# DHDev0/Stochastic-muzero

Hardware: NVIDIA B200
Metric: mcts_simulations_per_sec (higher is better)
Workload: dtype bf16

## Files before the change

### include/smz.h

```cpp
#ifndef SMZ_H_
#define SMZ_H_

#include <stddef.h>
#include <stdint.h>

#ifdef __cplusplus
extern "C" {
#endif

#define SMZ_ABI_VERSION 2

enum {
  SMZ_OK = 0,
  SMZ_E_INVALID_ARG = -1,
  SMZ_E_CUDA = -2,
  SMZ_E_CAPACITY = -3,
  SMZ_E_STATE = -4
};

enum {
  SMZ_NET_EXTERNAL = 0,
  SMZ_NET_FP32 = 1,
  SMZ_NET_BF16 = 2,
  SMZ_NET_TC32 = 4,
// ... 45 lines not shown
  uint64_t weight_blob_floats;
  uint64_t arena_bytes;
} smz_dims;

typedef struct smz_tree_host {
  int32_t* visit;
  float* value_sum;
  float* reward;
  float* prior;
  int32_t* child_base;
  int32_t* key;
  double* root_prior;
  float minmax[2];
  int32_t n_uniforms;
  int32_t root_to_play;
} smz_tree_host;

int smz_create(const smz_config* cfg, smz_engine** out);
int smz_destroy(smz_engine* e);
int smz_get_dims(const smz_engine* e, smz_dims* out);
const char* smz_last_error(void);

int smz_set_pbc_table(smz_engine* e, const double* table_host, int32_t n_entries);

int smz_set_player_tables(smz_engine* e, const int8_t* sign_host, const int32_t* to_play_host,
                          int32_t n_phases);

int smz_set_weights(smz_engine* e, const float* blob, uint64_t n_floats, int32_t on_device, void* stream);

int smz_set_seed(smz_engine* e, uint64_t seed, uint64_t tree_id_offset, void* stream);
// ... 37 lines not shown
```

### stochastic-muzero_b200/_lib.py

```python
import ctypes as C
import os

_HERE = os.path.dirname(os.path.abspath(__file__))
LIB_PATH = os.path.join(_HERE, "libsmz.so")

SMZ_ABI_VERSION = 2
SMZ_OK, SMZ_E_INVALID_ARG, SMZ_E_CUDA, SMZ_E_CAPACITY, SMZ_E_STATE = 0, -1, -2, -3, -4
NET_EXTERNAL, NET_FP32, NET_BF16, NET_VISION, NET_TC32, NET_F16 = 0, 1, 2, 3, 4, 5
RNG_PHILOX, RNG_TAPE = 0, 1


class smz_config(C.Structure):
    _fields_ = [
        ("abi_version", C.c_int32), ("device", C.c_int32), ("max_trees", C.c_int32),
        ("num_simulations", C.c_int32), ("action_dim", C.c_int32), ("chance_dim", C.c_int32),
        ("max_action_sample", C.c_int32), ("pb_c_base", C.c_int32),
        ("pb_c_init", C.c_double), ("discount", C.c_double), ("root_dirichlet_alpha", C.c_double),
        ("root_exploration_fraction", C.c_double),
        ("obs_dim", C.c_int32), ("state_dim", C.c_int32), ("hidden_dim", C.c_int32),
        ("num_hidden_layers", C.c_int32), ("net_mode", C.c_int32), ("rng_mode", C.c_int32),
        ("lanes_per_tree", C.c_int32), ("record", C.c_int32),
        ("seed", C.c_uint64), ("tree_id_offset", C.c_uint64),
    ]


class smz_dims(C.Structure):
    _fields_ = [
        ("nodes_per_tree", C.c_int32), ("max_children", C.c_int32), ("policy_stride", C.c_int32),
        ("hidden_stride", C.c_int32), ("hidden_slots", C.c_int32), ("path_stride", C.c_int32),
        ("lanes_per_tree", C.c_int32), ("reserved", C.c_int32),
        ("weight_blob_floats", C.c_uint64), ("arena_bytes", C.c_uint64),
    ]


class smz_tree_host(C.Structure):
    _fields_ = [
        ("visit", C.POINTER(C.c_int32)), ("value_sum", C.POINTER(C.c_float)), ("reward", C.POINTER(C.c_float)),
        ("prior", C.POINTER(C.c_float)), ("child_base", C.POINTER(C.c_int32)), ("key", C.POINTER(C.c_int32)),
        ("root_prior", C.POINTER(C.c_double)), ("minmax", C.c_float * 2), ("n_uniforms", C.c_int32),
        ("root_to_play", C.c_int32),
    ]


_P = C.c_void_p
SIGNATURES = {
    "smz_create": (C.c_int, [C.POINTER(smz_config), C.POINTER(_P)]),
    "smz_destroy": (C.c_int, [_P]),
    "smz_get_dims": (C.c_int, [_P, C.POINTER(smz_dims)]),
    "smz_last_error": (C.c_char_p, []),
    "smz_set_pbc_table": (C.c_int, [_P, C.POINTER(C.c_double), C.c_int32]),
    "smz_set_player_tables": (C.c_int, [_P, C.POINTER(C.c_int8), C.POINTER(C.c_int32), C.c_int32]),
    "smz_set_weights": (C.c_int, [_P, _P, C.c_uint64, C.c_int32, _P]),
    "smz_set_seed": (C.c_int, [_P, C.c_uint64, C.c_uint64, _P]),
    "smz_set_uniform_tape": (C.c_int, [_P, _P, C.c_int32]),
    "smz_root": (C.c_int, [_P, C.c_int32, _P, _P, _P, C.c_int32, _P, _P]),
# ... 32 lines not shown
```

### stochastic-muzero_b200/csrc/smz_api.cu

```cuda
#include <cuda_runtime.h>
#include <math.h>
#include <stdarg.h>
#include <stdio.h>
#include <stdlib.h>
#include <string.h>

#include <vector>

#include "../../include/smz.h"
#include "smz_kernels.h"
#include "smz_net_bf16.h"
#include "smz_net_tc32.h"
#include "smz_net_vision.h"

static thread_local char g_err[512] = "";

static int fail(int code, const char* fmt, ...) {
  va_list ap;
  va_start(ap, fmt);
  vsnprintf(g_err, sizeof(g_err), fmt, ap);
  va_end(ap);
  return code;
}

// ... 138 lines not shown
  a.one_minus_frac_f32 = (float)(1.0 - c.root_exploration_fraction);
  a.frac = c.root_exploration_fraction;
  a.alpha = c.root_dirichlet_alpha;

  e->dims.nodes_per_tree = a.M; e->dims.max_children = a.Kmax; e->dims.policy_stride = a.W;
  e->dims.hidden_stride = a.Sp; e->dims.hidden_slots = a.N + 1; e->dims.path_stride = a.path_stride;
  e->dims.lanes_per_tree = lanes;
  e->cfg.lanes_per_tree = lanes;

  const size_t B = a.B, M = a.M;
  a.row_cap = (a.B + 511) / 512 * 512 + 512;
  a.row_top = a.row_cap;
  const size_t RC = a.row_cap;
  cudaError_t r = cudaSuccess;
#define ALLOC(ptr, n) if (r == cudaSuccess) r = dev_alloc(e, &(ptr), (n))
  ALLOC(a.stat, B * M); ALLOC(a.link, B * M); ALLOC(a.root_prior, B * a.A); ALLOC(a.minmax, B);
  ALLOC(a.ucursor, B); ALLOC(a.root_to_play, B); ALLOC(a.path, B * a.path_stride); ALLOC(a.path_len, B);
  ALLOC(a.leaf_node, B); ALLOC(a.leaf_slot, B); ALLOC(a.leaf_action, B); ALLOC(a.leaf_branch, B);
  ALLOC(a.branch_count, (size_t)(a.N + 1) * 2); ALLOC(a.rows, 2 * RC); ALLOC(a.rows4, 2 * RC); ALLOC(a.error_flag, 1);
  ALLOC(a.depth_sum, 1);
  a.xin_q = c.net_mode == SMZ_NET_TC32 ? 16 : 8;
  if (c.net_mode == SMZ_NET_BF16 || c.net_mode == SMZ_NET_TC32 || c.net_mode == SMZ_NET_F16) { ALLOC(a.xin, 2 * RC * a.xin_q); }
  if (getenv("SMZ_TREE_TIMELINE")) { ALLOC(a.dbg, 8 + 4 * ((size_t)a.N + 2)); }
  ALLOC(a.out_policy, B * a.W); ALLOC(a.out_value, B); ALLOC(a.out_reward, B); ALLOC(a.dirichlet, B * a.A);
  if (c.record) {
    ALLOC(a.rec_policy, B * a.N * a.W); ALLOC(a.rec_value, B * a.N); ALLOC(a.rec_reward, B * a.N);
    ALLOC(a.rec_branch, B * a.N); ALLOC(a.rec_root_policy, B * a.W);
  }
  ALLOC(e->pbc_dev, (size_t)a.N + 2);
  ALLOC(e->rcp64_dev, (size_t)rcp_entries(a.N));
  ALLOC(e->rcp32_dev, (size_t)rcp_entries(a.N));
  ALLOC(e->seed_dev, 2);
  ALLOC(e->sign_dev, (size_t)a.N + 2);
  if (c.net_mode == SMZ_NET_VISION) {
    ALLOC(a.hidden, (size_t)(a.N + 1) * B * a.Sp);
    e->dims.weight_blob_floats = smz_vision_blob_floats(a.A, c.state_dim, c.hidden_dim, c.num_hidden_layers);
    ALLOC(e->blob_buf, e->dims.weight_blob_floats);
  } else if (c.net_mode != SMZ_NET_EXTERNAL) {
// ... 50 lines not shown
      double tree = 0, net = 0, g1 = 0, g2 = 0;
      int n = 0;
      for (int s = e->a.N - 11; s <= e->a.N - 2; ++s, ++n) {
        const unsigned long long *c = &w[4 * s], *nx = &w[4 * (s + 1)];
        net += (double)(c[3] - c[2]);
        g1 += (double)((long long)c[0] - (long long)c[3]);
        tree += (double)(c[1] - c[0]);
        g2 += (double)((long long)nx[2] - (long long)c[1]);
      }
      fprintf(stderr, "smz step timeline (%%globaltimer, mean of %d simulations): network step %.2f us | -> tree step %.2f us | tree step %.2f us | -> network step %.2f us\n",
              n, net / n / 1e3, g1 / n / 1e3, tree / n / 1e3, g2 / n / 1e3);
    }
    if (cudaMemcpy(t, e->a.dbg, sizeof(t), cudaMemcpyDeviceToHost) == cudaSuccess)
      fprintf(stderr, "smz tree timeline (block 0, last fused launch): expand+backup %lld cycles | descent %lld cycles = %lld levels walked by warp 0 in %lld + leaf record / row reservation %lld (path length of tree 0: %lld)\n",
              t[1] - t[0], t[2] - t[1], t[5], t[4] - t[1], t[2] - t[4], t[3]);
  }
  if (e->graph_exec) cudaGraphExecDestroy(e->graph_exec);
  if (e->capture_stream) cudaStreamDestroy(e->capture_stream);
  if (e->bf16) smz_bf16_destroy(e->bf16);
  if (e->tc32) smz_tc32_destroy(e->tc32);
  if (e->vision) smz_vision_destroy(e->vision);
  for (void* p : e->allocs) cudaFree(p);
  delete e;
  return SMZ_OK;
}

int smz_get_dims(const smz_engine* e, smz_dims* out) {
  if (!e || !out) return fail(SMZ_E_INVALID_ARG, "smz_get_dims: null argument");
  *out = e->dims;
  return SMZ_OK;
// ... 78 lines not shown

int smz_root(smz_engine* e, int32_t n_trees, const float* obs, const float* root_policy, const int32_t* root_to_play,
             int32_t train, const double* dirichlet, void* stream) {
  if (!e) return fail(SMZ_E_INVALID_ARG, "smz_root: null engine");
  if (n_trees < 1 || n_trees > e->a.B) return fail(SMZ_E_CAPACITY, "smz_root: n_trees %d not in [1, %d]", n_trees, e->a.B);
  if ((obs == nullptr) == (root_policy == nullptr))
    return fail(SMZ_E_INVALID_ARG, "smz_root: give exactly one of obs_dev / root_policy_dev");
  if (obs && e->cfg.net_mode == SMZ_NET_EXTERNAL) return fail(SMZ_E_STATE, "smz_root: obs given but engine has no network");
  if (obs && !e->have_weights) return fail(SMZ_E_STATE, "smz_root: smz_set_weights has not been called");
  if (e->cfg.rng_mode == SMZ_RNG_TAPE && !e->a.tape_u) return fail(SMZ_E_STATE, "smz_root: no uniform tape set");
  cudaStream_t s = (cudaStream_t)stream;
  ON_DEVICE(e);
  SmzArena& a = e->a;
  smz_launch_begin_search(a, s);
  if (a.dbg) {
    std::vector<unsigned long long> init(4 * ((size_t)a.N + 2));
    for (size_t i = 0; i < init.size(); ++i) init[i] = (i & 1) ? 0ull : ~0ull;
    CU(cudaMemcpyAsync(a.dbg + 8, init.data(), init.size() * sizeof(init[0]), cudaMemcpyHostToDevice, s));
    CU(cudaStreamSynchronize(s));
  }
  e->launches = 0;
  if (e->cfg.num_simulations == 0) train = 0;
  const float* policy = root_policy;
  if (obs) {
    if (e->vision) { smz_vision_root(e->vision, a, n_trees, obs, s); count_launches(e, 1); }
    else if (e->bf16) smz_bf16_root(e->bf16, a, e->shape, n_trees, obs, s);
    else if (e->tc32) smz_tc32_root(e->tc32, a, e->shape, n_trees, obs, s);
    else smz_net_f32_root(a, e->shape, e->img32, n_trees, obs, s);
    count_launches(e, 1);
    policy = a.out_policy;
  }
  if (train) {
// ... 187 lines not shown
  CU(cudaGetLastError());
  return SMZ_OK;
}

int smz_export_tree(smz_engine* e, int32_t tree, smz_tree_host* out, void* stream) {
  if (!e || !out) return fail(SMZ_E_INVALID_ARG, "smz_export_tree: null argument");
  if (tree < 0 || tree >= e->n_trees) return fail(SMZ_E_INVALID_ARG, "smz_export_tree: tree %d not in [0, %d)", tree, e->n_trees);
  ON_DEVICE(e);
  CU(cudaStreamSynchronize((cudaStream_t)stream));
  const SmzArena& a = e->a;
  const size_t M = a.M;
  std::vector<int4> stat(M);
  std::vector<int2> link(M);
  CU(cudaMemcpy(stat.data(), a.stat + (size_t)tree * M, M * sizeof(int4), cudaMemcpyDeviceToHost));
  CU(cudaMemcpy(link.data(), a.link + (size_t)tree * M, M * sizeof(int2), cudaMemcpyDeviceToHost));
  for (size_t n = 0; n < M; ++n) {
    if (out->visit) out->visit[n] = stat[n].x;
    if (out->value_sum) memcpy(&out->value_sum[n], &stat[n].y, 4);
    if (out->reward) memcpy(&out->reward[n], &stat[n].z, 4);
    if (out->prior) memcpy(&out->prior[n], &stat[n].w, 4);
    if (out->child_base) out->child_base[n] = link[n].x;
    if (out->key) out->key[n] = link[n].y;
  }
  if (out->root_prior)
    CU(cudaMemcpy(out->root_prior, a.root_prior + (size_t)tree * a.A, a.A * sizeof(double), cudaMemcpyDeviceToHost));
  float2 mm;
  CU(cudaMemcpy(&mm, a.minmax + tree, sizeof(mm), cudaMemcpyDeviceToHost));
  out->minmax[0] = mm.x; out->minmax[1] = mm.y;
  CU(cudaMemcpy(&out->n_uniforms, a.ucursor + tree, sizeof(int), cudaMemcpyDeviceToHost));
  CU(cudaMemcpy(&out->root_to_play, a.root_to_play + tree, sizeof(int), cudaMemcpyDeviceToHost));
// ... 56 lines not shown
```

### stochastic-muzero_b200/csrc/smz_common.cuh

```cuda
#pragma once
#include <cuda_runtime.h>
#include <stdint.h>

#define SMZ_BRANCH_AFTERSTATE 0
#define SMZ_BRANCH_DYNAMICS 1
#define SMZ_MAX_POLICY 32
#define SMZ_HP 128
#define SMZ_SP 64
#define SMZ_VISION_SP 160

struct SmzArena {
  int B, N, A, C, K, Kd, Kc, Kmax, M, W, Sp, path_stride, n_phases;
  int row_cap, row_top;
  int4* stat;
  int2* link;
  double* root_prior;
  float2* minmax;
  int* ucursor;
  int* root_to_play;
  int4* path;
  int* path_len;
  int* leaf_node;
  int* leaf_slot;
  int* leaf_action;
  int* leaf_branch;
  int* branch_count;
  int* rows;
  int4* rows4;
  uint4* xin;
  int xin_q;
// ... 18 lines not shown
  const double* rcp64;
  const float* rcp32;
  const signed char* sign;
  float discount;
  float one_minus_frac_f32;
  double frac;
  double alpha;
};

#ifdef __CUDACC__
__device__ __forceinline__ unsigned long long smz_globaltimer() {
  unsigned long long t;
  asm volatile("mov.u64 %0, %%globaltimer;" : "=l"(t));
  return t;
}
__device__ __forceinline__ void smz_stamp_min(long long* dbg, int sim, int k) {
  if (dbg && threadIdx.x == 0) atomicMin(reinterpret_cast<unsigned long long*>(dbg) + 8 + 4 * sim + k, smz_globaltimer());
}
__device__ __forceinline__ void smz_stamp_max(long long* dbg, int sim, int k) {
  if (dbg && threadIdx.x == 0) atomicMax(reinterpret_cast<unsigned long long*>(dbg) + 8 + 4 * sim + k, smz_globaltimer());
}
__device__ __forceinline__ size_t smz_row_index(const SmzArena& a, int sim, int branch, int row) {
  return (size_t)(sim & 1) * a.row_cap + (branch ? a.row_top - 1 - row : row);
}
__device__ __forceinline__ void smz_pdl_wait() { asm volatile("griddepcontrol.wait;" ::: "memory"); }
__device__ __forceinline__ void smz_pdl_launch_dependents() { asm volatile("griddepcontrol.launch_dependents;" ::: "memory"); }

template <typename... KArgs, typename... Args>
inline cudaError_t smz_launch(void (*kernel)(KArgs...), dim3 grid, dim3 block, size_t smem, cudaStream_t s, bool pdl,
                              Args... args) {
// ... 63 lines not shown
```

### stochastic-muzero_b200/csrc/smz_tree.cu

```cuda
#include <stdlib.h>

#include "smz_common.cuh"
#include "smz_kernels.h"
#include "smz_tree_dev.cuh"

namespace {

using namespace smz_tree_dev;

template <int G>
__global__ void k_root_expand(SmzArena a, int n_trees, const float* __restrict__ policy, int pstride,
                              const int* __restrict__ root_to_play, int train,
                              const double* __restrict__ dirichlet) {
  Group<G> g;
  int tree = (blockIdx.x * blockDim.x + threadIdx.x) / G;
  const bool alive = tree < n_trees;
  if (!alive) tree = n_trees - 1;
  const size_t tb = (size_t)tree * a.M;
  const int n = a.A;
  int cursor = 0;
  const float pol = (g.gl < n) ? policy[(size_t)tree * pstride + g.gl] : 0.f;
  const float p = normalise_policy(g, pol, n);
  const SmzRng rng = smz_make_rng(a);
  choice_without_replacement(g, a, rng, alive, tree, p, n, n, cursor);
  if (!alive) return;
  if (g.gl < n) {
    double prior = (double)p;
    if (train) {
      const double nz = dirichlet[(size_t)tree * a.A + g.gl];
      prior = __dadd_rn((double)__fmul_rn(p, a.one_minus_frac_f32), __dmul_rn(nz, a.frac));
    }
    a.root_prior[(size_t)tree * a.A + g.gl] = prior;
    a.stat[tb + 1 + g.gl] = make_int4(0, 0, 0, __float_as_int(p));
    a.link[tb + 1 + g.gl] = make_int2(0, g.gl);
  }
  if (g.gl == 0) {
    a.stat[tb] = make_int4(0, 0, 0, 0);
    a.link[tb] = make_int2(1, -1);
    a.minmax[tree] = make_float2(__int_as_float(0x7f800000), __int_as_float(0xff800000));
    a.ucursor[tree] = cursor;
    const int rtp = root_to_play ? root_to_play[tree] % a.n_phases : 0;
    a.root_to_play[tree] = rtp < 0 ? rtp + a.n_phases : rtp;
    a.path_len[tree] = 0;
    if (a.rec_root_policy)
      for (int i = 0; i < a.W; ++i) a.rec_root_policy[(size_t)tree * a.W + i] = i < n ? policy[(size_t)tree * pstride + i] : 0.f;
  }
}

template <int G>
__global__ void k_select(SmzArena a, int n_trees, int sim, int* __restrict__ o_slot, int* __restrict__ o_action,
                         int* __restrict__ o_branch) {
  Group<G> g;
// ... 8 lines not shown
  ts.root = make_int2(rs.x, rs.y);
  select_phase<G, true, false, true>(g, a, rng, tree, alive, sim, ts, o_slot, o_action, o_branch);
}

template <int G>
__global__ void k_expand_backup(SmzArena a, int n_trees, int sim, const float* __restrict__ policy, int pstride,
                                const float* __restrict__ value, const float* __restrict__ reward) {
  Group<G> g;
  int tree = (blockIdx.x * blockDim.x + threadIdx.x) / G;
  const bool alive = tree < n_trees;
  if (!alive) tree = n_trees - 1;
  const SmzRng rng = smz_make_rng(a);
  expand_backup_phase(g, a, rng, tree, alive, sim, policy, pstride, value, reward);
}

template <int G>
__global__ void k_backup_select(SmzArena a, int n_trees, int sim) {
  smz_pdl_wait();
  smz_pdl_launch_dependents();
  Group<G> g;
  int tree = (blockIdx.x * blockDim.x + threadIdx.x) / G;
  const bool alive = tree < n_trees;
  if (!alive) tree = n_trees - 1;
  const bool stamp = a.dbg && blockIdx.x == 0 && threadIdx.x == 0;
  if (stamp) a.dbg[0] = clock64();
  const SmzRng rng = smz_make_rng(a);
  const TreeState ts = expand_backup_phase(g, a, rng, tree, alive, sim, a.out_policy, a.W, a.out_value, a.out_reward);
  __syncwarp();
  if (stamp) a.dbg[1] = clock64();
  select_phase<G, true, false, true>(g, a, rng, tree, alive, sim + 1, ts, nullptr, nullptr, nullptr);
  if (stamp) { a.dbg[2] = clock64(); a.dbg[3] = a.path_len[tree]; }
}

constexpr int SMZ_UWIN = 32;

__host__ __device__ inline size_t smz_mirror_bytes(int tpb, int M, int A, int n_tab, int n_pbc) {
  size_t b = (size_t)tpb * M * (sizeof(int4) + sizeof(int2));
  b += (size_t)tpb * (A + SMZ_UWIN) * sizeof(double);
  b += (size_t)(n_pbc + n_tab) * sizeof(double) + (size_t)n_tab * sizeof(float);
  return b + 16;
}

template <int G>
__global__ void k_backup_select_sm(SmzArena a, int n_trees, int sim, int n_tab) {
  extern __shared__ int4 smz_sm_nodes[];
  Group<G> g;
  int tree = (blockIdx.x * blockDim.x + threadIdx.x) / G;
  const bool alive = tree < n_trees;
  if (!alive) tree = n_trees - 1;
  const int tpb = blockDim.x / G, lt = threadIdx.x / G;
  int4* sst = smz_sm_nodes + (size_t)lt * a.M;
  int2* slk_all = reinterpret_cast<int2*>(smz_sm_nodes + (size_t)tpb * a.M);
  int2* slk = slk_all + (size_t)lt * a.M;
  double* dbl = reinterpret_cast<double*>(slk_all + (size_t)tpb * a.M + ((size_t)tpb * a.M & 1));
  double* srp = dbl + (size_t)lt * a.A;
  double* swin = dbl + (size_t)tpb * a.A + (size_t)lt * SMZ_UWIN;
  double* spbc = dbl + (size_t)tpb * (a.A + SMZ_UWIN);
  double* sr64 = spbc + (a.N + 2);
  float* sr32 = reinterpret_cast<float*>(sr64 + n_tab);

  SmzRng rng = smz_make_rng(a);
  const int cursor0 = a.ucursor[tree];
  {
    const size_t tb = (size_t)tree * a.M;
    const int used = 1 + a.A + sim * a.Kmax;
    for (int i = g.gl; i < used; i += G) {
      sst[i] = a.stat[tb + i];
      slk[i] = a.link[tb + i];
    }
    for (int i = g.gl; i < a.A; i += G) srp[i] = a.root_prior[(size_t)tree * a.A + i];
    for (int i = threadIdx.x; i < a.N + 2; i += blockDim.x) spbc[i] = a.pbc[i];
    for (int i = threadIdx.x; i < n_tab; i += blockDim.x) { sr64[i] = a.rcp64[i]; sr32[i] = a.rcp32[i]; }
    if (rng.mode == 0)
      for (int i = g.gl; i < SMZ_UWIN; i += G) swin[i] = smz_rng_uniform(rng, tree, cursor0 + i);
  }
  SmzArena al = a;
  al.pbc = spbc; al.rcp64 = sr64; al.rcp32 = sr32;
  if (rng.mode == 0) { rng.win = swin; rng.win_base = cursor0; rng.win_len = SMZ_UWIN; }
  smz_pdl_wait();
  smz_pdl_launch_dependents();
  smz_stamp_min(a.dbg, sim, 0);
  __syncthreads();
  const bool stamp = a.dbg && blockIdx.x == 0 && threadIdx.x == 0;
  if (stamp) a.dbg[0] = clock64();
  const TreeState ts = expand_backup_phase<G, true>(g, al, rng, tree, alive, sim, a.out_policy, a.W, a.out_value, a.out_reward,
                                                    sst, slk);
  __syncwarp();
  if (stamp) a.dbg[1] = clock64();
  select_phase<G, true, true, true>(g, al, rng, tree, alive, sim + 1, ts, nullptr, nullptr, nullptr, sst, slk, srp);
  if (stamp) { a.dbg[2] = clock64(); a.dbg[3] = a.path_len[tree]; }
  if (a.dbg) {
    __syncthreads();
    smz_stamp_max(a.dbg, sim, 1);
  }
}

__global__ void k_read_roots(SmzArena a, int n_trees, int* __restrict__ visits, float* __restrict__ values,
                             double* __restrict__ priors, float* __restrict__ rewards, int* __restrict__ error_out) {
  const int i = blockIdx.x * blockDim.x + threadIdx.x;
  if (i == 0 && error_out) *error_out = *a.error_flag;
  if (i >= n_trees * a.A) return;
  const int tree = i / a.A, c = i % a.A;
  const size_t tb = (size_t)tree * a.M;
  const int4 st = a.stat[tb + 1 + c];
// ... 124 lines not shown
                              const float* value, const float* reward, cudaStream_t s) {
  SMZ_DISPATCH_G(lanes, (k_expand_backup<G><<<grid_for<G>(n_trees, kThreads), kThreads, 0, s>>>(
                            a, n_trees, sim, policy, pstride, value, reward)));
}

static int rcp_entries(const SmzArena& a) { return a.N + 3 > SMZ_MAX_POLICY + 1 ? a.N + 3 : SMZ_MAX_POLICY + 1; }
static size_t mirror_bytes(const SmzArena& a, int lanes) {
  return smz_mirror_bytes(kThreads / lanes, a.M, a.A, rcp_entries(a), a.N + 2);
}

bool smz_tree_mirror_fits(const SmzArena& a, int lanes) {
  const bool off = getenv("SMZ_NO_TREE_SMEM") != nullptr;
  return !off && mirror_bytes(a, lanes) <= 96 * 1024;
}

static bool mirror_pays(int blocks) {
  static int sms_of[64] = {0};
  int dev = 0;
  cudaGetDevice(&dev);
  int& sms = sms_of[dev & 63];
  if (!sms && (cudaDeviceGetAttribute(&sms, cudaDevAttrMultiProcessorCount, dev) != cudaSuccess || sms <= 0)) sms = 148;
  static const int per_sm = getenv("SMZ_MIRROR_BLOCKS_PER_SM") ? atoi(getenv("SMZ_MIRROR_BLOCKS_PER_SM")) : 2;
  return blocks <= per_sm * sms;
}

void smz_launch_backup_select(const SmzArena& a, int lanes, int n_trees, int sim, bool pdl, cudaStream_t s) {
  if (smz_tree_mirror_fits(a, lanes) && mirror_pays((n_trees * lanes + kThreads - 1) / kThreads)) {
    const size_t smem = mirror_bytes(a, lanes);
    SMZ_DISPATCH_G(lanes, (cudaFuncSetAttribute((const void*)k_backup_select_sm<G>, cudaFuncAttributeMaxDynamicSharedMemorySize,
                                                (int)smem),
                           getenv("SMZ_NO_CARVEOUT") ? cudaSuccess :
                           cudaFuncSetAttribute((const void*)k_backup_select_sm<G>, cudaFuncAttributePreferredSharedMemoryCarveout,
                                                cudaSharedmemCarveoutMaxShared),
                           smz_launch(k_backup_select_sm<G>, dim3(grid_for<G>(n_trees, kThreads)), dim3(kThreads), smem, s, pdl,
                                      a, n_trees, sim, rcp_entries(a))));
    return;
  }
  SMZ_DISPATCH_G(lanes, (smz_launch(k_backup_select<G>, dim3(grid_for<G>(n_trees, kThreads)), dim3(kThreads), 0, s, pdl,
                                    a, n_trees, sim)));
}

void smz_launch_read_roots(const SmzArena& a, int n_trees, int* visits, float* values, double* priors, float* rewards,
                           int* error_out, cudaStream_t s) {
  const int n = n_trees * a.A;
  k_read_roots<<<(n + 255) / 256, 256, 0, s>>>(a, n_trees, visits, values, priors, rewards, error_out);
}

void smz_launch_select_actions(const SmzArena& a, int n_trees, double temperature, const double* u, int* actions,
                               double* policy, double* stored, cudaStream_t s) {
  k_select_actions<<<(n_trees + 127) / 128, 128, 0, s>>>(a, n_trees, temperature, u, actions, policy, stored);
}

__global__ void k_begin_search(SmzArena a) {
  for (int i = threadIdx.x; i < (a.N + 1) * 2; i += blockDim.x) a.branch_count[i] = 0;
// ... 16 lines not shown
```

### stochastic-muzero_b200/csrc/smz_tree_dev.cuh

```cuda
#pragma once
#include "smz_common.cuh"

namespace smz_tree_dev {

#define FULL 0xffffffffu

template <int G>
struct Group {
  int lane, gl, gbase;
  __device__ Group() {
    lane = threadIdx.x & 31;
    gl = lane & (G - 1);
    gbase = lane & ~(G - 1);
  }
  template <typename T>
  __device__ T bcast(T v, int src) const { return __shfl_sync(FULL, v, src, G); }
  __device__ unsigned ballot(bool p) const {
    unsigned b = __ballot_sync(FULL, p);
    return (G == 32) ? b : ((b >> gbase) & ((1u << G) - 1u));
  }
};

template <int G>
__device__ float np_sum_f32(const Group<G>& g, float a, int n) {
// ... 97 lines not shown
#pragma unroll
      for (int i = 0; i < G; ++i) cnt += g.bcast(c, i) <= u;
    }
  }
  return cnt;
}

template <int G>
__device__ float normalise_policy(const Group<G>& g, float pol, int n) {
  const float p = (g.gl < n) ? __fadd_rn(pol, 1e-12f) : 0.f;
  const float s = np_sum_f32(g, p, n);
  return (g.gl < n) ? __fdiv_rn(p, s) : 0.f;
}

template <int G>
__device__ unsigned choice_without_replacement(const Group<G>& g, const SmzArena& a, const SmzRng& rng, bool alive, int tree,
                                               float p32, int n, int bound, int& cursor) {
  unsigned found = 0;
  int nf = alive ? 0 : bound;
  if (g.ballot(alive && g.gl < n && !(p32 >= 0.f))) {
    if (alive) *a.error_flag = 2;
    found = bound >= 32 ? 0xffffffffu : ((1u << bound) - 1u);
    nf = bound;
  }
  const double pd = (g.gl < n) ? (double)p32 : 0.0;
  for (int round = 0; __any_sync(FULL, nf < bound); ++round) {
    if (round > 2 * SMZ_MAX_POLICY) {
      if (nf < bound) {
        *a.error_flag = 2;
        for (int i = 0; i < n && nf < bound; ++i)
// ... 16 lines not shown
    for (int off = G / 2; off > 0; off >>= 1) bits |= __shfl_xor_sync(FULL, bits, off, G);
    found |= bits;
    nf = alive ? __popc(found) : bound;
    cursor += m;
  }
  return found;
}


struct TreeState {
  int cursor;
  float2 mm;
  int2 root;
};

template <int G, bool COMPACT = true, bool MIRROR = false, bool BLOCKAGG = false>
__device__ __forceinline__ void select_phase(const Group<G>& g, const SmzArena& a, const SmzRng& rng, int tree, bool alive,
                                             int sim, TreeState ts, int* __restrict__ o_slot, int* __restrict__ o_action,
                                             int* __restrict__ o_branch, const int4* __restrict__ sst = nullptr,
                                             const int2* __restrict__ slk = nullptr, const double* __restrict__ srp = nullptr) {
  const size_t tb = (size_t)tree * a.M;
  int cursor = ts.cursor;
  const float vmin = ts.mm.x, vmax = ts.mm.y;
  int4* path = a.path + (size_t)tree * a.path_stride;

  int depth = 0, cbase = 1, nch = a.A;
  int parent_visit = ts.root.x;
  const float range = __fsub_rn(vmax, vmin);
  const float rrange = vmax > vmin ? __frcp_rn(range) : 0.f;
  const bool range_plain = (__float_as_int(range) & 0x7FFFFF) == 0x7FFFFF || range < 1e-30f;
  if (alive && g.gl == 0) path[0] = make_int4(0, ts.root.x, ts.root.y, 0);
  int L = 1, child = 0, child_key = 0;
  bool going = alive;
  const double prior0 = (alive && g.gl < a.A) ? (srp ? srp[g.gl] : a.root_prior[(size_t)tree * a.A + g.gl]) : 0.0;
  int level = 0;
  while (__any_sync(FULL, going)) {
    const bool act = going && g.gl < nch;
    const bool chance = (level >> 1) & 1;
    const int ci = act ? cbase + g.gl : 0;
    int4 st;
    int2 lk;
    if constexpr (MIRROR) {
      st = sst[ci];
      lk = slk[ci];
    } else {
      st = a.stat[tb + ci];
      lk = a.link[tb + ci];
    }
    if (!act) { st = make_int4(0, 0, 0, 0); lk = make_int2(0, 0); }
    const double pbc = chance ? 0.0 : a.pbc[going ? parent_visit : 0];
    const int uidx = chance ? cursor : cursor + g.gl;
    const bool want = going && (chance || act);
    const unsigned wofs = (unsigned)(uidx - rng.win_base);
    const bool hit = rng.win != nullptr && wofs < (unsigned)rng.win_len;
    double u = hit ? rng.win[wofs] : 0.0;
    if (__any_sync(FULL, want && !hit)) {
      if (want && !hit) u = smz_rng_uniform(rng, tree, uidx);
    }
    int pick = 0;
    if (chance) {
      const float p = __int_as_float(st.w);
      const float om = act ? __fadd_rn(__fsub_rn(1.f, p), 1e-12f) : 0.f;
      const float rem = fabsf(smz_div_r32(np_sum_f32(g, om, nch), (float)nch, a.rcp32[nch]));
      const float sh = act ? __fadd_rn(p, rem) : 0.f;
      const float tot = np_sum_f32(g, sh, nch);
      const float q = act ? __fdiv_rn(sh, tot) : 0.f;
      double total;
      const double num = choice_cdf_raw(g, (double)q, nch, total);
      const float cf = cdf_f32(num, total, act), uf = (float)u;
      bool le = cf < uf;
      const bool close = act && fabsf(cf - uf) <= SMZ_CDF_MARGIN;
      if (__any_sync(FULL, close)) {
        if (close) le = __ddiv_rn(num, total) <= u;
      }
      int pk = __popc(g.ballot(act && le));
      pk = pk < nch ? pk : nch - 1;
      if (chance) { pick = pk; cursor += going ? 1 : 0; }
    }
    if (!chance) {
      double score = -__longlong_as_double(0x7ff0000000000000LL);
      int best = -1;
      if (act && !chance) {
        const double prior = (level == 0) ? prior0 : (double)__int_as_float(st.w);
        const double ps = smz_div_r64(__dmul_rn(pbc, prior), (double)(st.x + 1), a.rcp64[st.x + 1]);
        double vs = 0.0;
        if (st.x > 0) {
          const float val = smz_div_r32(__int_as_float(st.y), (float)st.x, a.rcp32[st.x]);
// ... 18 lines not shown
    const int key = g.bcast(lk.y, pick);
    if (going) {
      child = cbase + pick;
      child_key = key;
      if (g.gl == 0) path[L] = make_int4(child, cst.x, cst.y, cst.z);
      ++L;
      if (child_cb == 0 || L >= a.path_stride) {
        going = false;
      } else {
        nch = chance ? a.Kd : a.Kc;
        parent_visit = cst.x;
        cbase = child_cb;
        ++depth;
      }
    }
    ++level;
  }
  if (a.dbg && blockIdx.x == 0 && threadIdx.x == 0) { a.dbg[4] = clock64(); a.dbg[5] = level; }
  const bool lead = alive && g.gl == 0;
  const int branch = ((depth >> 1) & 1) ? SMZ_BRANCH_DYNAMICS : SMZ_BRANCH_AFTERSTATE;
  const int slot = (cbase == 1) ? 0 : (cbase - 1 - a.A) / a.Kmax + 1;
  uint4 hcopy[(G < 8) ? 8 / G : 1], hcopy2[(G < 8) ? 8 / G : 1];
  const bool copy_row = COMPACT && a.xin != nullptr && alive;
  const bool wide_row = a.xin_q > 8;
  if (copy_row) {
    const uint4* src = reinterpret_cast<const uint4*>(a.hidden) + ((size_t)slot * a.B + tree) * a.xin_q;
#pragma unroll
    for (int j = 0; j < ((G < 8) ? 8 / G : 1); ++j) {
      const int idx = g.gl + j * G;
      hcopy[j] = idx < 8 ? src[idx] : make_uint4(0, 0, 0, 0);
      if (wide_row) hcopy2[j] = idx < 8 ? src[8 + idx] : make_uint4(0, 0, 0, 0);
// ... 87 lines not shown
  float2 mm = a.minmax[tree];
  float v = value[tree];
  const float rew_in = reward[tree];
  const signed char* sign = a.sign + (size_t)a.root_to_play[tree] * (a.N + 2);

  const int n = branch ? a.A : a.C;
  const int bound = min(a.K, n);
  const float pol = (g.gl < n) ? policy[(size_t)tree * pstride + g.gl] : 0.f;
  const float p = normalise_policy(g, pol, n);
  const unsigned found = choice_without_replacement(g, a, rng, alive, tree, p, n, bound, cursor);
  const int cb = 1 + a.A + sim * a.Kmax;
  if (alive && g.gl < n && ((found >> g.gl) & 1u)) {
    const int r = __popc(found & ((1u << g.gl) - 1u));
    a.stat[tb + cb + r] = make_int4(0, 0, 0, __float_as_int(p));
    a.link[tb + cb + r] = make_int2(0, g.gl);
    if constexpr (MIRROR) {
      sst[cb + r] = make_int4(0, 0, 0, __float_as_int(p));
      slk[cb + r] = make_int2(0, g.gl);
    }
  }
  const float rew = branch ? rew_in : 0.f;
  if (alive && g.gl == 0) {
    a.link[tb + leaf].x = cb;
    a.ucursor[tree] = cursor;
    if (branch) reinterpret_cast<int*>(a.stat + tb + leaf)[2] = __float_as_int(rew);
    if constexpr (MIRROR) {
      slk[leaf].x = cb;
      if (branch) sst[leaf].z = __float_as_int(rew);
    }
    if (a.rec_policy) {
// ... 67 lines not shown
```

### stochastic-muzero_b200/engine.py

```python
from __future__ import annotations

import ctypes as C
from typing import Dict, Optional

import numpy as np
import torch

from . import _lib
from .weights import VISION_FLAT, ModelShape, VisionShape

SEARCH_KEYS = ("pb_c_base", "pb_c_init", "discount", "root_dirichlet_alpha", "root_exploration_fraction",
               "num_simulations", "maxium_action_sample", "number_of_player", "custom_loop")
_NET = {"external": _lib.NET_EXTERNAL, "fp32": _lib.NET_FP32, "bf16": _lib.NET_BF16, "vision": _lib.NET_VISION,
        "tc32": _lib.NET_TC32, "f16": _lib.NET_F16}
_RNG = {"philox": _lib.RNG_PHILOX, "tape": _lib.RNG_TAPE}


class SmzError(RuntimeError):
    pass


def _is_chance(depth: int) -> bool:
    return bool((depth >> 1) & 1)

# ... 273 lines not shown
               "dirichlet": self._new(n, A, dtype=torch.float64), "root_policy": self._new(n, W, dtype=torch.float32)}
        self._check(self.lib.smz_read_record(self._h, self._ptr(rec["sim_policy"]), self._ptr(rec["sim_value"]),
                                             self._ptr(rec["sim_reward"]), self._ptr(rec["sim_branch"]),
                                             self._ptr(rec["dirichlet"]), self._ptr(rec["root_policy"]), self._stream))
        return rec

    def stats(self):
        depth, launches, total = C.c_double(), C.c_int64(), C.c_int64()
        self._check(self.lib.smz_stats(self._h, C.byref(depth), C.byref(launches), C.byref(total), self._stream))
        return {"mean_leaf_depth": depth.value, "launches": launches.value, "launches_total": total.value}

    def export_arena(self, tree: int) -> Dict[str, np.ndarray]:
        M, A = self.dims.nodes_per_tree, self.A
        cols = {"visit": np.zeros(M, np.int32), "value_sum": np.zeros(M, np.float32), "reward": np.zeros(M, np.float32),
                "prior": np.zeros(M, np.float32), "child_base": np.zeros(M, np.int32), "key": np.zeros(M, np.int32),
                "root_prior": np.zeros(A, np.float64)}
        th = _lib.smz_tree_host()
        th.visit = cols["visit"].ctypes.data_as(C.POINTER(C.c_int32))
        th.value_sum = cols["value_sum"].ctypes.data_as(C.POINTER(C.c_float))
        th.reward = cols["reward"].ctypes.data_as(C.POINTER(C.c_float))
        th.prior = cols["prior"].ctypes.data_as(C.POINTER(C.c_float))
        th.child_base = cols["child_base"].ctypes.data_as(C.POINTER(C.c_int32))
        th.key = cols["key"].ctypes.data_as(C.POINTER(C.c_int32))
        th.root_prior = cols["root_prior"].ctypes.data_as(C.POINTER(C.c_double))
        self._check(self.lib.smz_export_tree(self._h, int(tree), C.byref(th), self._stream))
        cols["minmax"] = np.array([th.minmax[0], th.minmax[1]], np.float32)
        cols["n_uniforms"] = int(th.n_uniforms)
        cols["root_to_play"] = int(th.root_to_play)
        return cols

    def n_children(self, depth: int) -> int:
        if depth == 0:
            return self.A
        return min(self.K, self.A) if _is_chance(depth - 1) else min(self.K, self.Cdim)

    def export_tree(self, tree: int) -> Dict[str, np.ndarray]:
        ar = self.export_arena(tree)
        phase = ar["root_to_play"] % self.n_phases
        rows = []
# ... 17 lines not shown
```

Baseline: 187.3 million.

## Precompute and store chance-node CDFs instead of recomputing per descent

Adds a per-node cdf array. On expansion each chance child set gets a marker, and a fill pass at the start of backup_select computes the normalized chance CDF once. Later descents read the stored value instead of redoing two group reductions and a scan at every chance level. Values close to the margin are still recomputed exactly, and a heuristic picks the stored path only when the lane count or block count suggests it pays. The change also adds per-level timeline instrumentation behind the debug flag, plus extra memory and writes for the cdf array.

Result: faster. 190.3 million (median of 6 runs) (+1.6%).

```diff
diff --git a/include/smz.h b/include/smz.h
--- a/include/smz.h
+++ b/include/smz.h
@@ -83,6 +83,7 @@
   float minmax[2];
   int32_t n_uniforms;
   int32_t root_to_play;
+  float* cdf;
 } smz_tree_host;
 
 int smz_create(const smz_config* cfg, smz_engine** out);
diff --git a/stochastic-muzero_b200/_lib.py b/stochastic-muzero_b200/_lib.py
--- a/stochastic-muzero_b200/_lib.py
+++ b/stochastic-muzero_b200/_lib.py
@@ -38,7 +38,7 @@
         ("visit", C.POINTER(C.c_int32)), ("value_sum", C.POINTER(C.c_float)), ("reward", C.POINTER(C.c_float)),
         ("prior", C.POINTER(C.c_float)), ("child_base", C.POINTER(C.c_int32)), ("key", C.POINTER(C.c_int32)),
         ("root_prior", C.POINTER(C.c_double)), ("minmax", C.c_float * 2), ("n_uniforms", C.c_int32),
-        ("root_to_play", C.c_int32),
+        ("root_to_play", C.c_int32), ("cdf", C.POINTER(C.c_float)),
     ]
 
 
diff --git a/stochastic-muzero_b200/csrc/smz_api.cu b/stochastic-muzero_b200/csrc/smz_api.cu
--- a/stochastic-muzero_b200/csrc/smz_api.cu
+++ b/stochastic-muzero_b200/csrc/smz_api.cu
@@ -176,14 +176,14 @@
   const size_t RC = a.row_cap;
   cudaError_t r = cudaSuccess;
 #define ALLOC(ptr, n) if (r == cudaSuccess) r = dev_alloc(e, &(ptr), (n))
-  ALLOC(a.stat, B * M); ALLOC(a.link, B * M); ALLOC(a.root_prior, B * a.A); ALLOC(a.minmax, B);
+  ALLOC(a.stat, B * M); ALLOC(a.link, B * M); ALLOC(a.cdf, B * M); ALLOC(a.root_prior, B * a.A); ALLOC(a.minmax, B);
   ALLOC(a.ucursor, B); ALLOC(a.root_to_play, B); ALLOC(a.path, B * a.path_stride); ALLOC(a.path_len, B);
   ALLOC(a.leaf_node, B); ALLOC(a.leaf_slot, B); ALLOC(a.leaf_action, B); ALLOC(a.leaf_branch, B);
   ALLOC(a.branch_count, (size_t)(a.N + 1) * 2); ALLOC(a.rows, 2 * RC); ALLOC(a.rows4, 2 * RC); ALLOC(a.error_flag, 1);
   ALLOC(a.depth_sum, 1);
   a.xin_q = c.net_mode == SMZ_NET_TC32 ? 16 : 8;
   if (c.net_mode == SMZ_NET_BF16 || c.net_mode == SMZ_NET_TC32 || c.net_mode == SMZ_NET_F16) { ALLOC(a.xin, 2 * RC * a.xin_q); }
-  if (getenv("SMZ_TREE_TIMELINE")) { ALLOC(a.dbg, 8 + 4 * ((size_t)a.N + 2)); }
+  if (getenv("SMZ_TREE_TIMELINE")) { ALLOC(a.dbg, smz_tl_levels_base(a) + 8 * ((size_t)a.N + 2)); }
   ALLOC(a.out_policy, B * a.W); ALLOC(a.out_value, B); ALLOC(a.out_reward, B); ALLOC(a.dirichlet, B * a.A);
   if (c.record) {
     ALLOC(a.rec_policy, B * a.N * a.W); ALLOC(a.rec_value, B * a.N); ALLOC(a.rec_reward, B * a.N);
@@ -264,6 +264,12 @@
     if (cudaMemcpy(t, e->a.dbg, sizeof(t), cudaMemcpyDeviceToHost) == cudaSuccess)
       fprintf(stderr, "smz tree timeline (block 0, last fused launch): expand+backup %lld cycles | descent %lld cycles = %lld levels walked by warp 0 in %lld + leaf record / row reservation %lld (path length of tree 0: %lld)\n",
               t[1] - t[0], t[2] - t[1], t[5], t[4] - t[1], t[2] - t[4], t[3]);
+    unsigned long long q[8];
+    if (e->a.N >= 2 && cudaMemcpy(q, e->a.dbg + smz_tl_levels_base(e->a) + 8 * (e->a.N - 1), sizeof(q), cudaMemcpyDeviceToHost) == cudaSuccess &&
+        q[4] > 0)
+      fprintf(stderr, "smz tree levels (descent of simulation %d, all %llu warps): decision %.0f cycles/level over %llu levels | chance %.0f cycles/level over %llu levels | mean %.2f levels per warp | deepest warp %llu levels | slowest warp descent %llu cycles\n",
+              e->a.N - 1, q[4], q[1] ? (double)q[0] / q[1] : 0.0, q[1], q[3] ? (double)q[2] / q[3] : 0.0, q[3],
+              (double)(q[1] + q[3]) / q[4], q[5], q[6]);
   }
   if (e->graph_exec) cudaGraphExecDestroy(e->graph_exec);
   if (e->capture_stream) cudaStreamDestroy(e->capture_stream);
@@ -372,8 +378,8 @@
   SmzArena& a = e->a;
   smz_launch_begin_search(a, s);
   if (a.dbg) {
-    std::vector<unsigned long long> init(4 * ((size_t)a.N + 2));
-    for (size_t i = 0; i < init.size(); ++i) init[i] = (i & 1) ? 0ull : ~0ull;
+    std::vector<unsigned long long> init(12 * ((size_t)a.N + 2), 0ull);
+    for (size_t i = 0; i < 4 * ((size_t)a.N + 2); ++i) init[i] = (i & 1) ? 0ull : ~0ull;
     CU(cudaMemcpyAsync(a.dbg + 8, init.data(), init.size() * sizeof(init[0]), cudaMemcpyHostToDevice, s));
     CU(cudaStreamSynchronize(s));
   }
@@ -591,6 +597,7 @@
   std::vector<int2> link(M);
   CU(cudaMemcpy(stat.data(), a.stat + (size_t)tree * M, M * sizeof(int4), cudaMemcpyDeviceToHost));
   CU(cudaMemcpy(link.data(), a.link + (size_t)tree * M, M * sizeof(int2), cudaMemcpyDeviceToHost));
+  if (out->cdf) CU(cudaMemcpy(out->cdf, a.cdf + (size_t)tree * M, M * sizeof(float), cudaMemcpyDeviceToHost));
   for (size_t n = 0; n < M; ++n) {
     if (out->visit) out->visit[n] = stat[n].x;
     if (out->value_sum) memcpy(&out->value_sum[n], &stat[n].y, 4);
diff --git a/stochastic-muzero_b200/csrc/smz_common.cuh b/stochastic-muzero_b200/csrc/smz_common.cuh
--- a/stochastic-muzero_b200/csrc/smz_common.cuh
+++ b/stochastic-muzero_b200/csrc/smz_common.cuh
@@ -14,6 +14,7 @@
   int row_cap, row_top;
   int4* stat;
   int2* link;
+  float* cdf;
   double* root_prior;
   float2* minmax;
   int* ucursor;
@@ -62,6 +63,7 @@
   asm volatile("mov.u64 %0, %%globaltimer;" : "=l"(t));
   return t;
 }
+__host__ __device__ __forceinline__ size_t smz_tl_levels_base(const SmzArena& a) { return 8 + 4 * ((size_t)a.N + 2); }
 __device__ __forceinline__ void smz_stamp_min(long long* dbg, int sim, int k) {
   if (dbg && threadIdx.x == 0) atomicMin(reinterpret_cast<unsigned long long*>(dbg) + 8 + 4 * sim + k, smz_globaltimer());
 }
diff --git a/stochastic-muzero_b200/csrc/smz_tree.cu b/stochastic-muzero_b200/csrc/smz_tree.cu
--- a/stochastic-muzero_b200/csrc/smz_tree.cu
+++ b/stochastic-muzero_b200/csrc/smz_tree.cu
@@ -33,9 +33,11 @@
     a.root_prior[(size_t)tree * a.A + g.gl] = prior;
     a.stat[tb + 1 + g.gl] = make_int4(0, 0, 0, __float_as_int(p));
     a.link[tb + 1 + g.gl] = make_int2(0, g.gl);
+    a.cdf[tb + 1 + g.gl] = p;
   }
   if (g.gl == 0) {
     a.stat[tb] = make_int4(0, 0, 0, 0);
+    a.cdf[tb] = 0.f;
     a.link[tb] = make_int2(1, -1);
     a.minmax[tree] = make_float2(__int_as_float(0x7f800000), __int_as_float(0xff800000));
     a.ucursor[tree] = cursor;
@@ -74,21 +76,22 @@
   expand_backup_phase(g, a, rng, tree, alive, sim, policy, pstride, value, reward);
 }
 
-template <int G>
+template <int G, bool STORED>
 __global__ void k_backup_select(SmzArena a, int n_trees, int sim) {
+  Group<G> g;
+  int tree = (blockIdx.x * blockDim.x + threadIdx.x) / G;
+  const bool alive = tree < n_trees;
+  if (!alive) tree = n_trees - 1;
+  if (STORED) fill_chance_cdf(g, a, tree, alive, sim);
   smz_pdl_wait();
   smz_pdl_launch_dependents();
-  Group<G> g;
-  int tree = (blockIdx.x * blockDim.x + threadIdx.x) / G;
-  const bool alive = tree < n_trees;
-  if (!alive) tree = n_trees - 1;
   const bool stamp = a.dbg && blockIdx.x == 0 && threadIdx.x == 0;
   if (stamp) a.dbg[0] = clock64();
   const SmzRng rng = smz_make_rng(a);
   const TreeState ts = expand_backup_phase(g, a, rng, tree, alive, sim, a.out_policy, a.W, a.out_value, a.out_reward);
   __syncwarp();
   if (stamp) a.dbg[1] = clock64();
-  select_phase<G, true, false, true>(g, a, rng, tree, alive, sim + 1, ts, nullptr, nullptr, nullptr);
+  select_phase<G, true, false, true, STORED>(g, a, rng, tree, alive, sim + 1, ts, nullptr, nullptr, nullptr);
   if (stamp) { a.dbg[2] = clock64(); a.dbg[3] = a.path_len[tree]; }
 }
 
@@ -101,7 +104,7 @@
   return b + 16;
 }
 
-template <int G>
+template <int G, bool STORED>
 __global__ void k_backup_select_sm(SmzArena a, int n_trees, int sim, int n_tab) {
   extern __shared__ int4 smz_sm_nodes[];
   Group<G> g;
@@ -124,8 +127,12 @@
   {
     const size_t tb = (size_t)tree * a.M;
     const int used = 1 + a.A + sim * a.Kmax;
+    if (STORED) fill_chance_cdf(g, a, tree, alive, sim);
+    __syncwarp();
     for (int i = g.gl; i < used; i += G) {
-      sst[i] = a.stat[tb + i];
+      int4 st = a.stat[tb + i];
+      if (STORED) st.w = __float_as_int(a.cdf[tb + i]);
+      sst[i] = st;
       slk[i] = a.link[tb + i];
     }
     for (int i = g.gl; i < a.A; i += G) srp[i] = a.root_prior[(size_t)tree * a.A + i];
@@ -147,7 +154,7 @@
                                                     sst, slk);
   __syncwarp();
   if (stamp) a.dbg[1] = clock64();
-  select_phase<G, true, true, true>(g, al, rng, tree, alive, sim + 1, ts, nullptr, nullptr, nullptr, sst, slk, srp);
+  select_phase<G, true, true, true, STORED>(g, al, rng, tree, alive, sim + 1, ts, nullptr, nullptr, nullptr, sst, slk, srp);
   if (stamp) { a.dbg[2] = clock64(); a.dbg[3] = a.path_len[tree]; }
   if (a.dbg) {
     __syncthreads();
@@ -302,30 +309,41 @@
   return !off && mirror_bytes(a, lanes) <= 96 * 1024;
 }
 
-static bool mirror_pays(int blocks) {
+static int device_sms() {
   static int sms_of[64] = {0};
   int dev = 0;
   cudaGetDevice(&dev);
   int& sms = sms_of[dev & 63];
   if (!sms && (cudaDeviceGetAttribute(&sms, cudaDevAttrMultiProcessorCount, dev) != cudaSuccess || sms <= 0)) sms = 148;
+  return sms;
+}
+static bool mirror_pays(int blocks) {
   static const int per_sm = getenv("SMZ_MIRROR_BLOCKS_PER_SM") ? atoi(getenv("SMZ_MIRROR_BLOCKS_PER_SM")) : 2;
-  return blocks <= per_sm * sms;
-}
-
-void smz_launch_backup_select(const SmzArena& a, int lanes, int n_trees, int sim, bool pdl, cudaStream_t s) {
-  if (smz_tree_mirror_fits(a, lanes) && mirror_pays((n_trees * lanes + kThreads - 1) / kThreads)) {
+  return blocks <= per_sm * device_sms();
+}
+static bool stored_cdf_pays(int lanes, int blocks) { return lanes >= 16 || 2 * blocks <= 3 * device_sms(); }
+
+template <bool STORED>
+static void launch_backup_select(const SmzArena& a, int lanes, int n_trees, int sim, bool pdl, int blocks, cudaStream_t s) {
+  if (smz_tree_mirror_fits(a, lanes) && mirror_pays(blocks)) {
     const size_t smem = mirror_bytes(a, lanes);
-    SMZ_DISPATCH_G(lanes, (cudaFuncSetAttribute((const void*)k_backup_select_sm<G>, cudaFuncAttributeMaxDynamicSharedMemorySize,
+    SMZ_DISPATCH_G(lanes, (cudaFuncSetAttribute((const void*)k_backup_select_sm<G, STORED>, cudaFuncAttributeMaxDynamicSharedMemorySize,
                                                 (int)smem),
                            getenv("SMZ_NO_CARVEOUT") ? cudaSuccess :
-                           cudaFuncSetAttribute((const void*)k_backup_select_sm<G>, cudaFuncAttributePreferredSharedMemoryCarveout,
+                           cudaFuncSetAttribute((const void*)k_backup_select_sm<G, STORED>, cudaFuncAttributePreferredSharedMemoryCarveout,
                                                 cudaSharedmemCarveoutMaxShared),
-                           smz_launch(k_backup_select_sm<G>, dim3(grid_for<G>(n_trees, kThreads)), dim3(kThreads), smem, s, pdl,
+                           smz_launch(k_backup_select_sm<G, STORED>, dim3(grid_for<G>(n_trees, kThreads)), dim3(kThreads), smem, s, pdl,
                                       a, n_trees, sim, rcp_entries(a))));
     return;
   }
-  SMZ_DISPATCH_G(lanes, (smz_launch(k_backup_select<G>, dim3(grid_for<G>(n_trees, kThreads)), dim3(kThreads), 0, s, pdl,
+  SMZ_DISPATCH_G(lanes, (smz_launch(k_backup_select<G, STORED>, dim3(grid_for<G>(n_trees, kThreads)), dim3(kThreads), 0, s, pdl,
                                     a, n_trees, sim)));
+}
+
+void smz_launch_backup_select(const SmzArena& a, int lanes, int n_trees, int sim, bool pdl, cudaStream_t s) {
+  const int blocks = (n_trees * lanes + kThreads - 1) / kThreads;
+  if (stored_cdf_pays(lanes, blocks)) launch_backup_select<true>(a, lanes, n_trees, sim, pdl, blocks, s);
+  else launch_backup_select<false>(a, lanes, n_trees, sim, pdl, blocks, s);
 }
 
 void smz_launch_read_roots(const SmzArena& a, int n_trees, int* visits, float* values, double* priors, float* rewards,
diff --git a/stochastic-muzero_b200/csrc/smz_tree_dev.cuh b/stochastic-muzero_b200/csrc/smz_tree_dev.cuh
--- a/stochastic-muzero_b200/csrc/smz_tree_dev.cuh
+++ b/stochastic-muzero_b200/csrc/smz_tree_dev.cuh
@@ -135,6 +135,33 @@
 }
 
 template <int G>
+__device__ float chance_cdf(const Group<G>& g, const SmzArena& a, float p, bool act, int nch, double& num, double& total) {
+  const float om = act ? __fadd_rn(__fsub_rn(1.f, p), 1e-12f) : 0.f;
+  const float rem = fabsf(smz_div_r32(np_sum_f32(g, om, nch), (float)nch, a.rcp32[nch]));
+  const float sh = act ? __fadd_rn(p, rem) : 0.f;
+  const float tot = np_sum_f32(g, sh, nch);
+  const float q = act ? __fdiv_rn(sh, tot) : 0.f;
+  num = choice_cdf_raw(g, (double)q, nch, total);
+  return cdf_f32(num, total, act);
+}
+
+template <int G>
+__device__ __forceinline__ void fill_chance_cdf(const Group<G>& g, const SmzArena& a, int tree, bool alive, int sim) {
+  if (sim < 1) return;
+  const size_t at = (size_t)tree * a.M + 1 + a.A + (size_t)(sim - 1) * a.Kmax;
+  const bool in = g.gl < a.Kmax;
+  const float m = in ? a.cdf[at + g.gl] : 0.f;
+  const float p = in ? __int_as_float(a.stat[at + g.gl].w) : 0.f;
+  const float m0 = g.bcast(m, 0);
+  const int n = m0 < 0.f ? (int)(-m0) : 0;
+  const bool act = alive && g.gl < n;
+  if (!__any_sync(FULL, act)) return;
+  double num, total;
+  const float cf = chance_cdf(g, a, p, act, n, num, total);
+  if (act) a.cdf[at + g.gl] = cf;
+}
+
+template <int G>
 __device__ unsigned choice_without_replacement(const Group<G>& g, const SmzArena& a, const SmzRng& rng, bool alive, int tree,
                                                float p32, int n, int bound, int& cursor) {
   unsigned found = 0;
@@ -181,7 +208,7 @@
   int2 root;
 };
 
-template <int G, bool COMPACT = true, bool MIRROR = false, bool BLOCKAGG = false>
+template <int G, bool COMPACT = true, bool MIRROR = false, bool BLOCKAGG = false, bool STORED = false>
 __device__ __forceinline__ void select_phase(const Group<G>& g, const SmzArena& a, const SmzRng& rng, int tree, bool alive,
                                              int sim, TreeState ts, int* __restrict__ o_slot, int* __restrict__ o_action,
                                              int* __restrict__ o_branch, const int4* __restrict__ sst = nullptr,
@@ -201,20 +228,26 @@
   bool going = alive;
   const double prior0 = (alive && g.gl < a.A) ? (srp ? srp[g.gl] : a.root_prior[(size_t)tree * a.A + g.gl]) : 0.0;
   int level = 0;
+  const bool tl = a.dbg != nullptr;
+  long long tl_cd = 0, tl_cc = 0, tl_t0 = tl ? clock64() : 0, tl_t = tl_t0;
+  int tl_nd = 0, tl_nc = 0;
   while (__any_sync(FULL, going)) {
     const bool act = going && g.gl < nch;
     const bool chance = (level >> 1) & 1;
     const int ci = act ? cbase + g.gl : 0;
     int4 st;
     int2 lk;
+    float w = 0.f;
     if constexpr (MIRROR) {
       st = sst[ci];
       lk = slk[ci];
+      w = __int_as_float(st.w);
     } else {
       st = a.stat[tb + ci];
       lk = a.link[tb + ci];
-    }
-    if (!act) { st = make_int4(0, 0, 0, 0); lk = make_int2(0, 0); }
+      if (STORED && chance) w = a.cdf[tb + ci];
+    }
+    if (!act) { st = make_int4(0, 0, 0, 0); lk = make_int2(0, 0); w = 0.f; }
     const double pbc = chance ? 0.0 : a.pbc[going ? parent_visit : 0];
     const int uidx = chance ? cursor : cursor + g.gl;
     const bool want = going && (chance || act);
@@ -226,18 +259,28 @@
     }
     int pick = 0;
     if (chance) {
-      const float p = __int_as_float(st.w);
-      const float om = act ? __fadd_rn(__fsub_rn(1.f, p), 1e-12f) : 0.f;
-      const float rem = fabsf(smz_div_r32(np_sum_f32(g, om, nch), (float)nch, a.rcp32[nch]));
-      const float sh = act ? __fadd_rn(p, rem) : 0.f;
-      const float tot = np_sum_f32(g, sh, nch);
-      const float q = act ? __fdiv_rn(sh, tot) : 0.f;
-      double total;
-      const double num = choice_cdf_raw(g, (double)q, nch, total);
-      const float cf = cdf_f32(num, total, act), uf = (float)u;
+      const float uf = (float)u;
+      double num, total;
+      float cf, p = __int_as_float(st.w);
+      const bool fresh = cbase == 1 + a.A + (sim - 1) * a.Kmax;
+      if constexpr (STORED) {
+        const bool need = act && (fresh || w < 0.f);
+        cf = act ? w : 3.f;
+        if (__any_sync(FULL, need)) {
+          if (MIRROR && need && !fresh) p = __int_as_float(a.stat[tb + ci].w);
+          const float c = chance_cdf(g, a, p, need, nch, num, total);
+          if (need) cf = c;
+        }
+      } else {
+        cf = chance_cdf(g, a, p, act, nch, num, total);
+      }
       bool le = cf < uf;
       const bool close = act && fabsf(cf - uf) <= SMZ_CDF_MARGIN;
       if (__any_sync(FULL, close)) {
+        if constexpr (STORED) {
+          if (MIRROR && act && !fresh) p = __int_as_float(a.stat[tb + ci].w);
+          chance_cdf(g, a, p, act, nch, num, total);
+        }
         if (close) le = __ddiv_rn(num, total) <= u;
       }
       int pk = __popc(g.ballot(act && le));
@@ -286,7 +329,22 @@
         ++depth;
       }
     }
+    if (tl) {
+      const long long t = clock64();
+      if (chance) { tl_cc += t - tl_t; ++tl_nc; } else { tl_cd += t - tl_t; ++tl_nd; }
+      tl_t = t;
+    }
     ++level;
+  }
+  if (tl && level > 0 && (threadIdx.x & 31u) == 0) {
+    unsigned long long* q = reinterpret_cast<unsigned long long*>(a.dbg) + smz_tl_levels_base(a) + 8 * sim;
+    atomicAdd(q + 0, (unsigned long long)tl_cd);
+    atomicAdd(q + 1, (unsigned long long)tl_nd);
+    atomicAdd(q + 2, (unsigned long long)tl_cc);
+    atomicAdd(q + 3, (unsigned long long)tl_nc);
+    atomicAdd(q + 4, 1ull);
+    atomicMax(q + 5, (unsigned long long)level);
+    atomicMax(q + 6, (unsigned long long)(tl_t - tl_t0));
   }
   if (a.dbg && blockIdx.x == 0 && threadIdx.x == 0) { a.dbg[4] = clock64(); a.dbg[5] = level; }
   const bool lead = alive && g.gl == 0;
@@ -404,6 +462,7 @@
     const int r = __popc(found & ((1u << g.gl) - 1u));
     a.stat[tb + cb + r] = make_int4(0, 0, 0, __float_as_int(p));
     a.link[tb + cb + r] = make_int2(0, g.gl);
+    a.cdf[tb + cb + r] = ((L - 1) >> 1) & 1 ? -(float)__popc(found) : p;
     if constexpr (MIRROR) {
       sst[cb + r] = make_int4(0, 0, 0, __float_as_int(p));
       slk[cb + r] = make_int2(0, g.gl);
diff --git a/stochastic-muzero_b200/engine.py b/stochastic-muzero_b200/engine.py
--- a/stochastic-muzero_b200/engine.py
+++ b/stochastic-muzero_b200/engine.py
@@ -311,7 +311,7 @@
         M, A = self.dims.nodes_per_tree, self.A
         cols = {"visit": np.zeros(M, np.int32), "value_sum": np.zeros(M, np.float32), "reward": np.zeros(M, np.float32),
                 "prior": np.zeros(M, np.float32), "child_base": np.zeros(M, np.int32), "key": np.zeros(M, np.int32),
-                "root_prior": np.zeros(A, np.float64)}
+                "root_prior": np.zeros(A, np.float64), "cdf": np.zeros(M, np.float32)}
         th = _lib.smz_tree_host()
         th.visit = cols["visit"].ctypes.data_as(C.POINTER(C.c_int32))
         th.value_sum = cols["value_sum"].ctypes.data_as(C.POINTER(C.c_float))
@@ -320,6 +320,7 @@
         th.child_base = cols["child_base"].ctypes.data_as(C.POINTER(C.c_int32))
         th.key = cols["key"].ctypes.data_as(C.POINTER(C.c_int32))
         th.root_prior = cols["root_prior"].ctypes.data_as(C.POINTER(C.c_double))
+        th.cdf = cols["cdf"].ctypes.data_as(C.POINTER(C.c_float))
         self._check(self.lib.smz_export_tree(self._h, int(tree), C.byref(th), self._stream))
         cols["minmax"] = np.array([th.minmax[0], th.minmax[1]], np.float32)
         cols["n_uniforms"] = int(th.n_uniforms)
```
